# stvmsq/soc_project_stereo_matching

Hardware: AMD Instinct MI355X
Metric: Mdisp/s (W*H*D*paths/s; t_frame incl. H2D + D2H) (higher is better)
Workload: dtype u8

## Files before the change

### soc_project_stereo_matching_amd/csrc/sgm_aggregate_impl.hpp

```cpp
#pragma once
#include "sgm_common.hpp"

#ifndef SGM_AGG_PF
#define SGM_AGG_PF 2
#endif
#ifndef SGM_ANOM_PF
#define SGM_ANOM_PF 4
#endif
#ifndef SGM_AGG_HBURST
#define SGM_AGG_HBURST 1
#endif
#ifndef SGM_AGG_PF_HL
#define SGM_AGG_PF_HL 4
#endif


struct AggArgs {
    const uint8_t* img;
    const uint32_t* census_l;
    const uint32_t* census_r;
    const uint8_t* cost;
    int dmin;
    const uint16_t* lut;
    uint8_t* planes;
// ... 146 lines not shown
static __device__ __forceinline__ us2 pk_min_tree(const us2 (&v)[N])
{
    if constexpr (!FAST || N < 3) {
        us2 m = v[0];
#pragma unroll
        for (int j = 1; j < N; ++j) m = pk_min(m, v[j]);
        return m;
    } else {
        us2 m = pk_min3_f16(v[0], v[1], v[2]);
        int j = 3;
#pragma unroll
        for (; j + 1 < N; j += 2) m = pk_min3_f16(m, v[j], v[j + 1]);
        if (j < N) m = pk_min(m, v[j]);
        return m;
    }
}
template <int LPP>
static __device__ __forceinline__ unsigned row_allmin_pk(us2 m)
{
    unsigned r;
    asm("v_pk_min_u16 %0, %1, %1 op_sel:[0,1] op_sel_hi:[1,0]" : "=v"(r) : "v"(as_u(m)));
    return row_allmin<LPP>(r);
}
template <int DPL, bool PAD, int LPP, bool FAST = false>
static __device__ __forceinline__ unsigned agg_step_nn(unsigned cl, const CensusVec<DPL>& cv, int lim, bool border,
                                                       us2 (&Lp)[DPL / 2], unsigned mp, unsigned pen16, us2 p1v,
                                                       const us2 (&padmask)[DPL / 2], bool first_lane, bool last_lane,
                                                       unsigned (&sent)[2], CellVec<DPL>& packed_out)
{
    constexpr int NP = DPL / 2;
    const us2 p2v = as_p(pen16);
    const unsigned p1u = as_u(p1v);
    unsigned from_left, from_right;
    if (LPP >= 32) {
        from_left = sent[0] = dpp_mov<0x138 >(sent[0], as_u(Lp[NP - 1]));
        from_right = sent[1] = dpp_mov<0x130 >(sent[1], as_u(Lp[0]));
    } else {
        from_left = sent[0] = dpp_mov<DPP_ROW_SHR1>(sent[0], as_u(Lp[NP - 1]));
        from_right = sent[1] = dpp_mov<DPP_ROW_SHL1>(sent[1], as_u(Lp[0]));
    }
    if (LPP != 16) {
        from_left = first_lane ? 0x00FF00FFu : from_left;
        from_right = last_lane ? 0x00FF00FFu : from_right;
    }
    unsigned w[NP], md[NP];
#pragma unroll
    for (int j = 0; j < NP; ++j) {
        const unsigned below = (j == 0) ? from_left : as_u(Lp[j - 1]);
        const unsigned above = (j == NP - 1) ? from_right : as_u(Lp[j + 1]);
        const us2 dm1 = as_p(__builtin_amdgcn_alignbit(as_u(Lp[j]), below, 16) + p1u);
        const us2 dp1 = as_p(__builtin_amdgcn_alignbit(above, as_u(Lp[j]), 16) + p1u);
        us2 m;
        if constexpr (FAST) m = pk_min3_f16(dm1, dp1, Lp[j]);
        else m = pk_min(pk_min(dm1, dp1), Lp[j]);
        md[j] = as_u(pk_min(as_p(as_u(m) - mp), p2v));
        const unsigned lo = bcnt_acc(cl ^ cv.r[DPL - 1 - 2 * j], md[j]);
        w[j] = shl16_add((unsigned)__popc(cl ^ cv.r[DPL - 2 - 2 * j]), lo);
    }
    if (border) {
#pragma unroll
        for (int j = 0; j < NP; ++j) {
            const unsigned msk = (2 * j > lim ? 0xFFFFu : 0u) | (2 * j + 1 > lim ? 0xFFFF0000u : 0u);
            w[j] = (w[j] & ~msk) | ((md[j] + 0x007F007Fu) & msk);
            if constexpr (FAST) w[j] &= 0x00FF00FFu;
        }
    }
    us2 Ln[NP];
#pragma unroll
    for (int j = 0; j < NP; ++j) {
        unsigned r = w[j];
        if constexpr (!FAST) r &= 0x00FF00FFu;
        if (PAD) r |= as_u(padmask[j]);
        Ln[j] = as_p(r);
    }
    const us2 m = pk_min_tree<NP, FAST>(Ln);
#pragma unroll
    for (int j = 0; j < NP; ++j) Lp[j] = Ln[j];
    pack_cells<DPL>(Ln, packed_out);
    return row_allmin_pk<LPP>(m);
}

enum { AGG_H = 0, AGG_V = 1, AGG_D = 2 };

template <int DPL, bool PAD, int LPP, int KIND, int NN, bool WIDE = false, bool VOL = false, bool PWO = false>
static __device__ __forceinline__ void agg_regular(const AggArgs& a, const AggFrame& fr, const unsigned short* lut_s,
                                                   const unsigned* lut32_s, int dir, int grp)
{
    constexpr int NP = DPL / 2;
    constexpr int PF = (LPP >= 32) ? SGM_AGG_PF_HL : SGM_AGG_PF;
    const int lane = threadIdx.x;
    const int dx = a.dx[dir], dy = a.dy[dir];
    const int W = a.W, H = a.H, Dp = a.Dp;
    const bool fwd = (dx == 1 && dy == 0) || (dx == 0 && dy == 1) || (dx == 1 && dy == 1) || (dx == -1 && dy == 1);
    const int s = fwd ? 1 : -1;
    const int rows = a.row_end - a.row_begin;
    const int skip = (KIND == AGG_H) ? 0 : (fwd ? a.row_begin : H - a.row_end);
    const bool import_state = skip > 0;
    const int nlines = (KIND == AGG_H) ? rows : a.line_lo[dir] + a.line_n[dir];
    constexpr bool pwo = PWO;
    bool wrapped = false;
    const int nsteps = (KIND == AGG_H) ? W - 1 : (import_state ? rows : rows - 1);
    if (KIND == AGG_D && W < 2) return;

    constexpr int LPW = 64 / LPP;
    const int sub = lane & (LPP - 1);
    const bool first_lane = (sub == 0), last_lane = (sub == LPP - 1);
    int line = ((KIND == AGG_H) ? 0 : a.line_lo[dir]) + grp * LPW + lane / LPP;
    bool store_ok = line < nlines;
    if (!store_ok) line = nlines - 1;
    if (KIND == AGG_D && line == a.anom_line[dir]) {
        store_ok = false;
        line = (line == 0) ? 1 : line - 1;
    }
    const unsigned lane_off = (unsigned)(sub * DPL);
    uint8_t* const plane = fr.planes + (size_t)dir * a.plane_bytes;

    us2 padmask[NP];
#pragma unroll
    for (int j = 0; j < NP; ++j) {
        const unsigned lo = ((int)lane_off + 2 * j >= a.D) ? 0x00FFu : 0u;
        const unsigned hi = ((int)lane_off + 2 * j + 1 >= a.D) ? 0x00FF0000u : 0u;
        padmask[j] = as_p(lo | hi);
    }

    unsigned p, off;
    int x;
    unsigned rowpix = 0, rowoff = 0, pcol = 0, col = 0;
    int dstep_p = 0, dstep_off = 0;
    if (KIND == AGG_H) {
        x = fwd ? 0 : W - 1;
        p = (unsigned)((a.row_begin + line) * W + x);
        dstep_p = s; dstep_off = s * Dp;
    } else if (KIND == AGG_V) {
        x = line;
        const int r = fwd ? a.row_begin - (import_state ? 1 : 0) : a.row_end - 1 + (import_state ? 1 : 0);
        p = (unsigned)(r * W + line);
        dstep_p = s * W; dstep_off = s * W * Dp;
    } else {
        rowpix = (unsigned)(fwd ? 0 : (H - 1) * W);
        rowoff = rowpix * (unsigned)Dp;
        pcol = col = (unsigned)line;
        x = line;
        p = rowpix + pcol;
        dstep_p = s * W; dstep_off = s * W * Dp;
    }
    off = p * (unsigned)Dp + lane_off;
    const int col_step = (dx == dy) ? s : -s;
    const unsigned wrap_at = (col_step > 0) ? (unsigned)(W - 1) : 0u, wrap_to = (col_step > 0) ? 0u : (unsigned)(W - 1);
    const unsigned pstep_n = (unsigned)(dstep_p + col_step), pstep_w = (unsigned)(dstep_p - col_step * (W - 1));
    const unsigned ostep_n = pstep_n * (unsigned)Dp, ostep_w = pstep_w * (unsigned)Dp;
    const int back = a.dmin + (int)lane_off + DPL - 1;
    const int lim_bias = a.dmin + (int)lane_off;

    auto advance = [&]() {
        if (KIND == AGG_H) {
            p += (unsigned)dstep_p;
            off += (unsigned)dstep_off;
            x += s;
        } else if (KIND == AGG_V) {
            p += (unsigned)dstep_p;
            off += (unsigned)dstep_off;
        } else if (WIDE) {
            const bool wrap = (pcol == wrap_at);
            if constexpr (PWO) wrapped = wrapped || wrap;
            pcol = wrap ? wrap_to : pcol + (unsigned)col_step;
            p += wrap ? pstep_w : pstep_n;
            off += wrap ? ostep_w : ostep_n;
            x = (int)pcol;
        } else {
            const bool wr = (col == (unsigned)(W - 1));
            const bool wl = !wr && (col == 0);
            pcol = wr ? 0u : (wl ? (unsigned)(W - 1) : pcol + (unsigned)col_step);
            col = ((wr ? 0u : (wl ? (unsigned)(W - 1) : col)) + (unsigned)col_step) & 0xFFFFu;
            rowpix += (unsigned)dstep_p;
            rowoff += (unsigned)dstep_off;
            p = rowpix + pcol;
            x = (int)pcol;
            off = rowoff + __umul24(pcol, (unsigned)Dp) + lane_off;
        }
    };
    const unsigned cbias = (unsigned)(a.dmin + Dp - back);
    const char* const crb = reinterpret_cast<const char*>(fr.census_r - (a.dmin + Dp));
    const char* const clb_base = reinterpret_cast<const char*>(fr.census_l);
    auto fetch = [&](CensusVec<DPL>& cv, unsigned& cl, uint8_t& g) {
        if constexpr (VOL) {
            load_volume<DPL>(fr.cost + off, cv);
            cl = 0;
        } else {
            load_census<DPL>(reinterpret_cast<const uint32_t*>(crb + (size_t)((p + cbias) << 2)), cv);
            cl = *reinterpret_cast<const uint32_t*>(clb_base + (size_t)(p << 2));
        }
        g = fr.img[p];
    };

    if (KIND == AGG_D)
        for (int i = 0; i + 1 < skip; ++i) advance();

    us2 Lp[NP];
    unsigned min_prev;
    int g_prev;
    if (import_state) {
        CellVec<DPL> c0;
        load_cells<DPL>(plane + off, c0);
        g_prev = fr.img[p];
#pragma unroll
        for (int j = 0; j < NP; ++j) {
            const unsigned w = c0.w[j >> 1];
            Lp[j] = as_p(__builtin_amdgcn_perm(w, w, (j & 1) ? 0x0c030c02u : 0x0c010c00u));
        }
        us2 m = Lp[0];
#pragma unroll
        for (int j = 1; j < NP; ++j) m = pk_min(m, Lp[j]);
        min_prev = row_allmin<LPP>(min(as_u(m) & 0xFFFFu, as_u(m) >> 16));
    } else {
        CensusVec<DPL> cv;
        unsigned cl;
        uint8_t g0;
        fetch(cv, cl, g0);
        g_prev = g0;
        const int lim = x - lim_bias;
        if constexpr (VOL) volume_costs<DPL>(cv, Lp);
        else census_costs<DPL>(cl, cv, lim, true, Lp);
        if (PAD) {
#pragma unroll
            for (int j = 0; j < NP; ++j) Lp[j] = as_p(as_u(Lp[j]) | as_u(padmask[j]));
        }
        us2 m = Lp[0];
#pragma unroll
        for (int j = 1; j < NP; ++j) m = pk_min(m, Lp[j]);
        min_prev = row_allmin<LPP>(min(as_u(m) & 0xFFFFu, as_u(m) >> 16));
        if (store_ok && !pwo) {
            CellVec<DPL> o;
            pack_cells<DPL>(Lp, o);
            store_cells<DPL>(plane + off, o);
        }
    }

    CensusVec<DPL> cb[PF];
    unsigned clb[PF];
    uint8_t gb[PF];
    int limb[PF];
    unsigned ob[PF];
    bool wb[PF];
#pragma unroll
    for (int u = 0; u < PF; ++u) {
        gb[u] = 0; ob[u] = off; clb[u] = 0; limb[u] = 0; wb[u] = false;
#pragma unroll
        for (int i = 0; i < DPL; ++i) cb[u].r[i] = 0;
        if (1 + u <= nsteps) {
            advance();
            ob[u] = off;
            if constexpr (PWO) wb[u] = wrapped;
            limb[u] = x - lim_bias;
            fetch(cb[u], clb[u], gb[u]);
        }
    }
    const us2 p1v = splat((unsigned)a.p1);
    unsigned sent[2] = {0x00FF00FFu, 0x00FF00FFu};
    if constexpr (NN) min_prev |= min_prev << 16;

    auto step = [&](int u, bool refill, CellVec<DPL>* defer = nullptr, unsigned* defer_o = nullptr) {
        const int g = (int)gb[u];
        const int lim = limb[u];
        const unsigned o = ob[u];
        const bool st_ok = store_ok && (!pwo || wb[u]);
        const unsigned dg = __builtin_amdgcn_sad_u8((unsigned)g, (unsigned)g_prev, 0u);
        CellVec<DPL> packed;
        if constexpr (NN) {
            min_prev = agg_step_nn<DPL, PAD, LPP, NN == 2>(clb[u], cb[u], lim, __any(lim < DPL - 1) != 0, Lp, min_prev, lut32_s[dg], p1v,
                                                  padmask, first_lane, last_lane, sent, packed);
            if (refill) {
                advance();
                ob[u] = off;
                if constexpr (PWO) wb[u] = wrapped;
                limb[u] = x - lim_bias;
                fetch(cb[u], clb[u], gb[u]);
            }
        } else {
            us2 C[NP];
            if constexpr (VOL) volume_costs<DPL>(cb[u], C);
            else census_costs<DPL>(clb[u], cb[u], lim, __any(lim < DPL - 1) != 0, C);
            if (refill) {
                advance();
                ob[u] = off;
                if constexpr (PWO) wb[u] = wrapped;
                limb[u] = x - lim_bias;
                fetch(cb[u], clb[u], gb[u]);
            }
            min_prev = agg_step<DPL, PAD, LPP>(C, Lp, min_prev, lut_s[dg], p1v, padmask, first_lane, last_lane, packed);
        }
        g_prev = g;
        if (defer) { *defer = packed; *defer_o = o; }
        else if (st_ok) store_cells<DPL>(plane + o, packed);
    };
    __builtin_amdgcn_s_waitcnt(0x0F70);
    int k0 = 1;
    if constexpr (KIND == AGG_H && NN != 0 && SGM_AGG_HBURST > 1 && SGM_AGG_HBURST % PF == 0) {
        constexpr int HB = SGM_AGG_HBURST;
        for (; k0 + HB + PF - 1 <= nsteps; k0 += HB) {
            CellVec<DPL> pk[HB];
            unsigned po[HB];
#pragma unroll
            for (int j = 0; j < HB; ++j) step(j % PF, true, &pk[j], &po[j]);
            if (store_ok) {
#pragma unroll
                for (int j = 0; j < HB; ++j) store_cells<DPL>(plane + po[j], pk[j]);
            }
        }
    }
    for (; k0 + 2 * PF - 1 <= nsteps; k0 += PF) {
#pragma unroll
        for (int u = 0; u < PF; ++u) step(u, true);
    }
    for (; k0 <= nsteps; k0 += PF) {
#pragma unroll
        for (int u = 0; u < PF; ++u)
            if (k0 + u <= nsteps) step(u, k0 + u + PF <= nsteps);
    }
}

template <int DPL, bool PAD, int LPP, int NN, bool VOL = false>
static __device__ __forceinline__ void agg_anomalous(const AggArgs& a, const AggFrame& fr, const unsigned short* lut_s,
                                                     const unsigned* lut32_s, int dir)
{
    static_assert(!(NN && VOL), "the volume-fed lines run the generic step");
    constexpr int NP = DPL / 2;
    constexpr int NW = (DPL + 3) / 4;
    const int lane = threadIdx.x;
    const int dx = a.dx[dir], dy = a.dy[dir];
    const int W = a.W, H = a.H, Dp = a.Dp;
    const bool fwd = (dx == 1 && dy == 1) || (dx == -1 && dy == 1);
    const int s = fwd ? 1 : -1;
    const int diag_step = s * (W + ((dx == dy) ? 1 : -1));
    const int col_step = (dx == dy) ? s : -s;
    const int nsteps = H - 1;
    const long long npx = (long long)W * H;
    const int line = a.anom_line[dir];
    const int slot = dir - 4;
    const bool store_ok = lane < LPP;
    const int sub = lane & (LPP - 1);
    const bool first_lane = (sub == 0), last_lane = (sub == LPP - 1);
    const unsigned lane_off = (unsigned)(sub * DPL);
    uint8_t* const plane = fr.planes + (size_t)dir * a.plane_bytes;
    uint8_t* const extras = fr.extras + (size_t)slot * H * Dp + lane_off;

    us2 padmask[NP];
#pragma unroll
    for (int j = 0; j < NP; ++j) {
        const unsigned lo = ((int)lane_off + 2 * j >= a.D) ? 0x00FFu : 0u;
        const unsigned hi = ((int)lane_off + 2 * j + 1 >= a.D) ? 0x00FF0000u : 0u;
        padmask[j] = as_p(lo | hi);
    }
    auto ghost_zero = [&](int k) {
        if (store_ok && a.ghost_zero) {
            int gc = line + dx * k;
            if (gc >= W) gc -= W;
            if (gc < 0) gc += W;
            const int gr = fwd ? k : H - 1 - k;
            if (gr >= a.row_begin && gr < a.row_end) {
// ... 103 lines not shown
            if (refill) {
                advance();
                fetch(u);
            }
        } else {
            us2 C[NP];
            if constexpr (VOL) volume_costs<DPL>(cb[u], C);
            else census_costs<DPL>(clb[u], cb[u], limb[u], true, C);
            if (refill) {
                advance();
                fetch(u);
            }
            min_prev = agg_step<DPL, PAD, LPP>(C, Lp, min_prev, lut_s[dg], p1v, padmask, first_lane, last_lane, packed);
        }
        g_prev = g;
        if (store_ok) store_cells<DPL>(extras + (size_t)k * Dp, packed);
        ghost_zero(k);
    };
    __builtin_amdgcn_s_waitcnt(0x0F70);
    int k0 = 1;
    for (; k0 + 2 * PF - 1 <= n_live; k0 += PF) {
#pragma unroll
        for (int u = 0; u < PF; ++u) step(u, k0 + u, true);
    }
    for (; k0 <= n_live; k0 += PF) {
#pragma unroll
        for (int u = 0; u < PF; ++u)
            if (k0 + u <= n_live) step(u, k0 + u, k0 + u + PF <= n_live);
    }
    for (int k = n_live + 1; k <= nsteps; ++k) ghost_zero(k);
}

template <int DP> struct anom_layout   { static constexpr int lpp = (DP % 128 == 0) ? 64 : (DP == 64 ? 32 : 16), dpl = DP / lpp; };
template <int DP> struct anom_layout16 { static constexpr int lpp = 16, dpl = DP / 16; };

template <bool VOL>
static __device__ __forceinline__ AggFrame agg_frame(const AggArgs& a, int frame)
{
    AggFrame fr;
    fr.img = a.img + (size_t)frame * a.W * a.H;
    fr.census_l = a.census_l + (size_t)frame * a.W * a.H;
    fr.census_r = a.census_r + (size_t)frame * a.W * a.H;
    fr.cost = VOL ? a.cost + (size_t)frame * a.W * a.H * a.Dp : nullptr;
    fr.planes = a.planes + (size_t)frame * 8 * a.plane_bytes;
    fr.extras = a.extras + (size_t)frame * 4 * a.H * a.Dp;
    return fr;
}

template <int DPL, bool PAD, int LPP, int NN, bool VOL>
__global__ __launch_bounds__(64) void sgm_aggregate_anom_k(const AggArgs a)
{
    __shared__ unsigned short lut_s[256];
    __shared__ unsigned lut32_s[256];
    const int lane = threadIdx.x;
#pragma unroll
    for (int i = 0; i < 4; ++i) {
        const unsigned pen = a.lut[lane * 4 + i];
        lut_s[lane * 4 + i] = (unsigned short)pen;
        lut32_s[lane * 4 + i] = pen * 0x00010001u;
    }
    __syncthreads();
    const AggFrame fr = agg_frame<VOL>(a, blockIdx.x % a.B);
    agg_anomalous<DPL, PAD, LPP, NN, VOL>(a, fr, lut_s, lut32_s, 4 + blockIdx.x / a.B);
}
#ifdef SGM_CLOCK_PROBE
static __device__ unsigned long long g_sgm_agg_clock[2];
#endif

template <int DPL, bool PAD, int LPP, int HL, int NN, bool VOL = false>
__global__ __launch_bounds__(64) void sgm_aggregate_k(const AggArgs a)
{
#ifdef SGM_CLOCK_PROBE
    const unsigned long long clk0 = __builtin_amdgcn_s_memtime(), rt0 = __builtin_amdgcn_s_memrealtime();
    struct ClockProbe {
        unsigned long long c0, r0;
        __device__ ~ClockProbe() {
            if (blockIdx.x == 0 && threadIdx.x == 0) {
                g_sgm_agg_clock[0] = __builtin_amdgcn_s_memtime() - c0;
                g_sgm_agg_clock[1] = __builtin_amdgcn_s_memrealtime() - r0;
            }
        }
    } probe{clk0, rt0};
#endif
    __shared__ unsigned short lut_s[256];
    __shared__ unsigned lut32_s[256];
    const int lane = threadIdx.x;
#pragma unroll
    for (int i = 0; i < 4; ++i) {
        const unsigned pen = a.lut[lane * 4 + i];
        lut_s[lane * 4 + i] = (unsigned short)pen;
        lut32_s[lane * 4 + i] = pen * 0x00010001u;
    }
    __syncthreads();

    int frame, b;
    const int n_anom = a.anom_inline ? 4 : 0;
    if (a.strips > 1) {
        const int xcd = blockIdx.x & 7;
        frame = xcd % a.B;
        const int sub = xcd / a.B;
        int q = blockIdx.x >> 3;
        b = -1;
        for (int dd = 0; dd <= 8; ++dd) {
            const int d = dd == 0 ? 8 : dd - 1;
            const int begin = a.block_begin[d];
            const int n = (d < 8 ? a.block_begin[d + 1] : begin + n_anom) - begin;
            const int lo = sub * n / a.strips, share = (sub + 1) * n / a.strips - lo;
            if (q < share) { b = begin + lo + q; break; }
            q -= share;
        }
        if (b < 0) return;
    } else {
        frame = blockIdx.x % a.B;
        b = blockIdx.x / a.B;
        b = b < n_anom ? a.block_begin[8] + b : b - n_anom;
    }
    const AggFrame fr = agg_frame<VOL>(a, frame);
    if constexpr (NN != 0 && !VOL) {
        if (b >= a.block_begin[8]) {
            using AL = anom_layout<DPL * LPP>;
            agg_anomalous<AL::dpl, PAD, AL::lpp, 1, false>(a, fr, lut_s, lut32_s, 4 + (b - a.block_begin[8]));
            return;
        }
    }
    int dir = 0;
    while (dir + 1 < a.ndirs && b >= a.block_begin[dir + 1]) ++dir;
    const int grp = b - a.block_begin[dir];
    if (a.dy[dir] == 0) __builtin_amdgcn_s_setprio(3);
    if (a.dy[dir] == 0) {
        if constexpr (HL != 0) agg_regular<DPL * LPP / HL, PAD, HL, AGG_H, NN, false, VOL>(a, fr, lut_s, lut32_s, dir, grp);
        else               agg_regular<DPL, PAD, LPP, AGG_H, NN, false, VOL>(a, fr, lut_s, lut32_s, dir, grp);
    }
    else if (a.dx[dir] == 0) agg_regular<DPL, PAD, LPP, AGG_V, NN, false, VOL>(a, fr, lut_s, lut32_s, dir, grp);
    else if (a.W > a.H) {
        if constexpr (NN != 0 && !VOL) {
            if ((a.post_wrap_mask >> dir) & 1) {
                agg_regular<DPL, PAD, LPP, AGG_D, NN, true, VOL, true>(a, fr, lut_s, lut32_s, dir, grp);
                return;
            }
        }
        agg_regular<DPL, PAD, LPP, AGG_D, NN, true, VOL>(a, fr, lut_s, lut32_s, dir, grp);
    }
    else                     agg_regular<DPL, PAD, LPP, AGG_D, NN, false, VOL>(a, fr, lut_s, lut32_s, dir, grp);
}

template <int DPL, int LPP, int HL, int NN>
static bool launch_aggregate_hl(const AggArgs& a, int blocks, bool pad, hipStream_t st)
{
    constexpr int per = (HL != 0) ? DPL * LPP / HL : DPL;
    constexpr bool ok = (HL == 0) || ((DPL * LPP) % HL == 0 && (per == 2 || per == 4 || per == 8 || per == 16) && HL != LPP);
    if constexpr (ok) {
        if (pad) hipLaunchKernelGGL((sgm_aggregate_k<DPL, true, LPP, HL, NN>), dim3(blocks), dim3(64), 0, st, a);
        else     hipLaunchKernelGGL((sgm_aggregate_k<DPL, false, LPP, HL, NN>), dim3(blocks), dim3(64), 0, st, a);
        return true;
    }
    return false;
}
template <int DPL, int LPP, int NN>
static void launch_aggregate(const AggArgs& a, int blocks, bool pad, int hl, hipStream_t st)
{
    if constexpr (NN) {
        if (hl == 64 && launch_aggregate_hl<DPL, LPP, 64, NN>(a, blocks, pad, st)) return;
        if (hl == 32 && launch_aggregate_hl<DPL, LPP, 32, NN>(a, blocks, pad, st)) return;
        if (hl == 16 && launch_aggregate_hl<DPL, LPP, 16, NN>(a, blocks, pad, st)) return;
    }
    launch_aggregate_hl<DPL, LPP, 0, NN>(a, blocks, pad, st);
}

template <int NN>
static bool launch_aggregate_key(int lpp, int dpl, const AggArgs& a, int blocks, bool pad, int hl, hipStream_t st)
{
    switch (lpp * 100 + dpl) {
    case 1602: launch_aggregate<2, 16, NN>(a, blocks, pad, hl, st); return true;
    case 1604: launch_aggregate<4, 16, NN>(a, blocks, pad, hl, st); return true;
    case 1608: launch_aggregate<8, 16, NN>(a, blocks, pad, hl, st); return true;
    case 1612: launch_aggregate<12, 16, NN>(a, blocks, pad, hl, st); return true;
    case 1616: launch_aggregate<16, 16, NN>(a, blocks, pad, hl, st); return true;
    case 1632: launch_aggregate<32, 16, NN>(a, blocks, pad, hl, st); return true;
    default: break;
    }
    if constexpr (NN) {
        switch (lpp * 100 + dpl) {
        case 804: launch_aggregate<4, 8, NN>(a, blocks, pad, hl, st); return true;
        case 808: launch_aggregate<8, 8, NN>(a, blocks, pad, hl, st); return true;
        case 816: launch_aggregate<16, 8, NN>(a, blocks, pad, hl, st); return true;
        default: break;
        }
    }
    return false;
}
```

### soc_project_stereo_matching_amd/csrc/sgm_host.c

```c
#include "../../include/sgm_mi355x.h"
#include "sgm_device.h"

#include <math.h>
#include <stddef.h>
#include <stdio.h>
#include <stdlib.h>
#include <string.h>

#define SGM_VERSION_STRING "sgm_mi355x 0.3 (gfx950, hand-written HIP)"
#define CENSUS_FRONT_SLACK ((size_t)(65535 + SGM_MAX_DISPARITY_RANGE + 8 + 63) / 64 * 64 * 4)

#define TIMING_RING 64
enum { T_CENSUS, T_COST, T_AGGREGATE, T_SUM, T_WTA, T_LRCHECK, T_SPECKLE, T_MEDIAN, T_COUNT };
#define M_END T_COUNT
#define M_SUM_BEGIN (T_COUNT + 1)
#define MARKS_PER_MATCH (T_COUNT + 2)
static const char* const k_stage_names[T_COUNT] = {"census", "cost", "aggregate", "sum", "wta", "lrcheck", "speckle", "median"};

static const int k_dir_dx[8] = {1, -1, 0, 0, 1, -1, 1, -1};
static const int k_dir_dy[8] = {0, 0, 1, -1, 1, -1, -1, 1};

typedef struct { void* p; size_t cap; } sgm_buf;
typedef struct { void* dst; const void* src; size_t bytes; } handover;

typedef enum { S_ZERO, S_STORED, S_IN_PLANES, S_IN_PLANES_ADDS } sum_where;
typedef struct { sum_where where; bool up_missing; } sum_state;

typedef struct {
    float lambda, sigma;
    int iters, keep_invalid;
    float tab[SGM_REFINE_MAX_ITERS][256];
} refine_params;

struct sgm_instance {
    int device;
    void* stream;
    void* sum_stream;
    void* post_stream;
    void *ev_agg, *ev_sum, *ev_post;
    int overlap_post;
    bool sum_pending;
    bool post_pending;
    void* tail_stream;
    int cu_first[3], cu_count[3];
    int up_rows;
    sgm_buf d_up_scratch;
    sgm_buf d_left_keep;
    unsigned up_gen;
    int up_key[5];
    int last_up_rows;
    int env_upsum, env_upsum_rows, env_upsum_wgs;
    int env_lanes, env_hl, env_agg_fast, env_fused;
    bool stage_prio[3];
    int* h_status;
    void* timer;
    int timing;
    int keep_stages;
    int honor_num_paths;
    int census_w, census_h;
    int census_kind;
    int reference_view;
    int pixel_bits_req;
    int pixel_bits;
    int fill_req;
    bool fill_on;
    int refine_req;
    bool refine_on;
    int reference_statics;
    int batch;
    int read_frame;
    int tile_begin, tile_end;
    const void* tile_left;

    bool initialized;
    sum_state S;
    int fused_wta;
    SGMOption opt;
    sgmd_geom g;
    sgmd_paths paths;
    int need_plane_memset;
    int row_cap;
    float last_ms[T_COUNT];
    bool have_ms;
    int ring_next, ring_pending;
    double sum_ms[T_COUNT], min_ms[T_COUNT];
    long n_timed;

    int plane_row_lo, plane_rows;
    int tab_W, tab_H, tab_ndirs, tab_p1, tab_p2;
    sgm_buf d_left, d_right, d_census_l, d_census_r_alloc, d_cost, d_planes_alloc, d_extras, d_S;
    void *d_census_r, *d_planes;
    sgm_buf d_disp, d_disp_r, d_labels, d_sizes, d_lut, d_row_extras, d_row_count;
    sgm_buf d_snap_wta, d_snap_lr, d_snap_speckle, d_totals, d_median_scratch;
// ... 615 lines not shown
    const int bw = 64, bh = 16;
    for (int r = s->g.row_begin / bh; r <= (s->g.row_end - 1) / bh; ++r) memset(need + (size_t)r * bx, 1, (size_t)bx);
    if (s->paths.ndirs > 4) {
        const int back = s->g.dmin + s->g.Dp + 64;
        for (int d = 4; d < 8; ++d) {
            const int cnt = walk_line(W, H, k_dir_dx[d], k_dir_dy[d], s->paths.anom_line[d], pix);
            for (int k = 0; k < cnt; ++k) {
                const int y = pix[k] / W, x = pix[k] % W;
                const int c0 = (x - back < 0 ? 0 : x - back) / bw, c1 = x / bw;
                memset(need + (size_t)(y / bh) * bx + c0, 1, (size_t)(c1 - c0 + 1));
                if (x - back < 0 && y > 0) need[(size_t)((y - 1) / bh) * bx + bx - 1] = 1;
            }
        }
    }
    free(pix);
    const bool ok = reserve(s, &s->d_census_need, n, 0) && sgmd_h2d_async(s->device, s->stream, s->d_census_need.p, need, n) == 0 && sync_streams(s) == 0;
    free(need);
    if (!ok) FAIL("uploading the census block map failed");
    memcpy(s->need_key, key, sizeof key);
    return true;
}

#define ROW_EXTRAS_MAX ((size_t)1 << 24)

static bool upload_tables(sgm_instance* s)
{
    const int W = s->g.W, H = s->g.H;
    uint16_t lut[256];
    build_p2_table(s->opt.p1, s->opt.p2_init, lut);

    int32_t* pix = (int32_t*)malloc(sizeof(int32_t) * (size_t)(W > H ? W : H));
    int* count = (int*)calloc((size_t)H, sizeof(int));
    int32_t* visits = (int32_t*)malloc(sizeof(int32_t) * 4 * (size_t)H);
    if (!pix || !count || !visits) { free(pix); free(count); free(visits); FAIL("out of host memory"); }
    for (int i = 0; i < 4 * H; ++i) visits[i] = -1;
    if (s->paths.ndirs > 4) {
        for (int slot = 0; slot < 4; ++slot) {
            const int d = 4 + slot;
            const int n = walk_line(W, H, k_dir_dx[d], k_dir_dy[d], s->paths.anom_line[d], pix);
            for (int k = 0; k < n; ++k) {
                visits[slot * H + k] = pix[k];
                count[pix[k] / W]++;
            }
        }
    }
    int cap = 1;
    for (int r = 0; r < H; ++r) if (count[r] > cap) cap = count[r];
    if ((size_t)H * cap > ROW_EXTRAS_MAX) {
        free(pix); free(count); free(visits);
        FAIL("a frame %d wide and %d rows tall is not supported: its anomalous lines visit one row %d times (a frame one pixel wide "
             "is accepted up to 4096 rows)", W, H, cap);
    }
    sgmd_row_extra* table = (sgmd_row_extra*)calloc((size_t)H * cap, sizeof *table);
    if (!table) { free(pix); free(count); free(visits); FAIL("out of host memory"); }
    memset(count, 0, sizeof(int) * (size_t)H);
    for (int slot = 0; slot < 4; ++slot)
        for (int k = 0; k < H; ++k) {
            const int32_t p = visits[slot * H + k];
            if (p < 0) continue;
            const int r = p / W, c = p % W;
            table[(size_t)r * cap + count[r]].col_slot = c | (slot << 16);
            table[(size_t)r * cap + count[r]].step = k;
            count[r]++;
        }

    const buf_request tables[] = {{&s->d_row_extras, sizeof *table * (size_t)H * cap, 0}, {&s->d_row_count, sizeof(int) * (size_t)H, 0}};
    s->row_cap = cap;
    const bool ok = reserve_all(s, tables, 2, BUF_LAZY_DRAIN) && sgmd_h2d_async(s->device, s->stream, s->d_row_extras.p, table, sizeof *table * (size_t)H * cap) == 0 &&
         sgmd_h2d_async(s->device, s->stream, s->d_row_count.p, count, sizeof(int) * (size_t)H) == 0 &&
         sgmd_h2d_async(s->device, s->stream, s->d_lut.p, lut, sizeof lut) == 0 &&
         sync_streams(s) == 0;
    free(table); free(visits); free(count); free(pix);
    if (!ok) FAIL("uploading path tables failed");
    return true;
}

static bool ensure_buffers(sgm_instance* s)
{
    const int dev = s->device;
    const size_t px = batch_px(s);
    if (!buf_holds(&s->d_disp, px * 4)) {
        const size_t img = image_bytes(s);
        const buf_request images[] = {{&s->d_left, img, 0}, {&s->d_right, img, 0}, {&s->d_census_l, px * 4, 0},
                                      {&s->d_census_r_alloc, CENSUS_FRONT_SLACK + px * 4, 0}};
        const buf_request maps[] = {{&s->d_disp, px * 4, 0}, {&s->d_disp_r, px * 4, 0}, {&s->d_labels, px * 4, 0}, {&s->d_sizes, px * 4, 0},
                                    {&s->d_totals, px * 4, 0}, {&s->d_lut, 512, 0}, {&s->d_snap_wta, px * 4, 0}, {&s->d_snap_lr, px * 4, 0},
                                    {&s->d_snap_speckle, px * 4, 0}, {&s->h_left, img, BUF_PINNED}, {&s->h_right, img, BUF_PINNED},
                                    {&s->h_disp, px * 4, BUF_PINNED}};
        sync_streams(s);
        const sgm_buf old_l = s->d_census_l, old_r = s->d_census_r_alloc;
        s->d_census_l = s->d_census_r_alloc = (sgm_buf){NULL, 0};
        free_device_buffers(s);
        int rc = reserve_all(s, images, 4, BUF_LAZY_DRAIN) ? 0 : -1;
        if (rc == 0) s->d_census_r = (char*)s->d_census_r_alloc.p + CENSUS_FRONT_SLACK;
        if (rc == 0) rc |= sgmd_memset_async(dev, s->stream, s->d_census_l.p, 0, px * 4);
        if (rc == 0) rc |= sgmd_memset_async(dev, s->stream, s->d_census_r_alloc.p, 0, CENSUS_FRONT_SLACK + px * 4);
        if (rc == 0 && s->reference_statics && old_l.p && old_r.p) {
            rc |= sgmd_d2d_async(dev, s->stream, s->d_census_l.p, old_l.p, old_l.cap);
            rc |= sgmd_d2d_async(dev, s->stream, s->d_census_r, (char*)old_r.p + CENSUS_FRONT_SLACK, old_l.cap);
        }
        if (rc == 0) rc |= sgmd_stream_sync(dev, s->stream);
        sgmd_free(dev, old_l.p);
        sgmd_free(dev, old_r.p);
        if (rc != 0 || !reserve_all(s, maps, 12, BUF_LAZY_DRAIN)) {
            free_device_buffers(s);
            FAIL("device allocation failed for %dx%dx%d", s->g.W, s->g.H, s->g.D);
        }
    }
    if (wide_pixels(s)) {
        const size_t img = image_bytes(s);
        const buf_request wide[] = {{&s->d_left, img, 0}, {&s->d_right, img, 0}, {&s->h_left, img, BUF_PINNED}, {&s->h_right, img, BUF_PINNED},
                                    {&s->d_g8_l, px, 0}, {&s->d_g8_r, px, 0}};
        if (!reserve_all(s, wide, 6, 0)) FAIL("device allocation failed for the %d-bit images of %dx%d", s->pixel_bits, s->g.W, s->g.H);
    }
    const bool tiled = row_tiled(s);
    s->plane_row_lo = tiled && s->g.row_begin > 0 ? s->g.row_begin - 1 : 0;
    const int row_hi = tiled && s->g.row_end < s->g.H ? s->g.row_end + 1 : s->g.H;
    s->plane_rows = row_hi - s->plane_row_lo;
    s->plane_bytes = (size_t)s->plane_rows * s->g.W * s->g.Dp;
    const size_t need = (size_t)s->g.B * 8 * s->plane_bytes;
    if (!reserve(s, &s->d_planes_alloc, need, 0))
        FAIL("device allocation failed for the path-cost planes of %dx%dx%d (%zu bytes)", s->g.W, s->g.H, s->g.D, need);
    s->d_planes = (void*)((uintptr_t)s->d_planes_alloc.p - (uintptr_t)s->plane_row_lo * s->g.W * s->g.Dp);
    return true;
}

static int ensure_S(sgm_instance* s)
{
    const size_t need = batch_px(s) * s->g.Dp * 2;
    if (buf_holds(&s->d_S, need)) return 0;
    if (reserve(s, &s->d_S, need, BUF_ZERO) &&
        (!s->sum_stream || sgmd_stream_sync(s->device, s->stream) == 0))
        return 0;
    fprintf(stderr, "sgm_mi355x: device allocation failed for the aggregated-cost volume (%zu bytes)\n", need);
    return -1;
}

static int ensure_cost(sgm_instance* s)
{
    const size_t need = batch_px(s) * s->g.Dp;
    if (reserve(s, &s->d_cost, need, 0)) return 0;
    fprintf(stderr, "sgm_mi355x: device allocation failed for the cost volume (%zu bytes)\n", need);
    return -1;
}

static int ensure_fill(sgm_instance* s)
{
    const size_t px = batch_px(s);
    const buf_request maps[] = {{&s->d_fill_class, px, 0}, {&s->d_fill_map, px * sizeof(float), 0}};
    if (reserve_all(s, maps, 2, 0)) return 0;
    fprintf(stderr, "sgm_mi355x: device allocation failed for the hole-filling maps (%zu pixels)\n", px);
    return -1;
}

static int ensure_refine(sgm_instance* s)
{
    const size_t px = batch_px(s);
    const buf_request maps[] = {{&s->d_rf_u, px * 4, 0}, {&s->d_rf_v, px * 4, 0}, {&s->d_rf_q, px * 4, 0}, {&s->d_rf_conf, px * 2, 0},
                                {&s->d_rf_guide[0], px, 0}, {&s->d_rf_guide[1], px, 0}};
    if (reserve_all(s, maps, 6, 0)) return 0;
    fprintf(stderr, "sgm_mi355x: device allocation failed for the refinement maps (%zu pixels)\n", px);
    return -1;
}

static int refine_passes(sgm_instance* s, void* st, void* disp, const void* conf, const void* guide, const refine_params* p)
{
    int rc = 0;
// ... 1427 lines not shown
```

Baseline: 1.883 million.

## Share right-census window across lanes via LDS in vertical/diagonal aggregation

For vertical and wide-diagonal aggregation paths, each wave now cooperatively loads one contiguous run of right-image census words per step (one 16-byte vector per lane) into shared memory. Each lane then reads its DPL-wide disparity window from LDS instead of issuing its own overlapping global gathers. Diagonals that wrap across the image edge use a second run. The aim is to cut redundant global/L2 traffic for overlapping census windows. In exchange it adds LDS writes, reads and wave barriers per step, shrinks lut_s when NN is set, and needs extra back slack on the census buffer for over-reads.

Result: faster. 1.950 million (median of 6 runs) (+3.5%).

```diff
diff --git a/soc_project_stereo_matching_amd/csrc/sgm_aggregate_impl.hpp b/soc_project_stereo_matching_amd/csrc/sgm_aggregate_impl.hpp
--- a/soc_project_stereo_matching_amd/csrc/sgm_aggregate_impl.hpp
+++ b/soc_project_stereo_matching_amd/csrc/sgm_aggregate_impl.hpp
@@ -252,11 +252,21 @@
 
 enum { AGG_H = 0, AGG_V = 1, AGG_D = 2 };
 
+template <int DPL, int LPP> struct agg_feed {
+    static constexpr int LPW = 64 / LPP;
+    static constexpr int RUNW = (DPL * LPP + LPW + 2 + 3) & ~3;
+    static constexpr bool on = DPL >= 16 && LPP <= 16 && RUNW / 4 <= 64;
+    static constexpr int BASE_DOWN = 16;
+};
+
 template <int DPL, bool PAD, int LPP, int KIND, int NN, bool WIDE = false, bool VOL = false, bool PWO = false>
 static __device__ __forceinline__ void agg_regular(const AggArgs& a, const AggFrame& fr, const unsigned short* lut_s,
-                                                   const unsigned* lut32_s, int dir, int grp)
+                                                   const unsigned* lut32_s, unsigned* feed_s, int dir, int grp)
 {
     constexpr int NP = DPL / 2;
+    using FD = agg_feed<DPL, LPP>;
+    constexpr bool FEED = FD::on && NN != 0 && !VOL && !PWO && (KIND == AGG_V || (KIND == AGG_D && WIDE));
+    constexpr int NRUN = (KIND == AGG_D) ? 2 : 1;
     constexpr int PF = (LPP >= 32) ? SGM_AGG_PF_HL : SGM_AGG_PF;
     const int lane = threadIdx.x;
     const int dx = a.dx[dir], dy = a.dy[dir];
@@ -275,13 +285,15 @@
     constexpr int LPW = 64 / LPP;
     const int sub = lane & (LPP - 1);
     const bool first_lane = (sub == 0), last_lane = (sub == LPP - 1);
-    int line = ((KIND == AGG_H) ? 0 : a.line_lo[dir]) + grp * LPW + lane / LPP;
+    const int line0 = ((KIND == AGG_H) ? 0 : a.line_lo[dir]) + grp * LPW;
+    int line = line0 + lane / LPP;
     bool store_ok = line < nlines;
     if (!store_ok) line = nlines - 1;
     if (KIND == AGG_D && line == a.anom_line[dir]) {
         store_ok = false;
         line = (line == 0) ? 1 : line - 1;
     }
+    const int feed_col = line - line0 + 1;
     const unsigned lane_off = (unsigned)(sub * DPL);
     uint8_t* const plane = fr.planes + (size_t)dir * a.plane_bytes;
 
@@ -297,6 +309,7 @@
     int x;
     unsigned rowpix = 0, rowoff = 0, pcol = 0, col = 0;
     int dstep_p = 0, dstep_off = 0;
+    unsigned frow = 0, fcol = 0;
     if (KIND == AGG_H) {
         x = fwd ? 0 : W - 1;
         p = (unsigned)((a.row_begin + line) * W + x);
@@ -306,6 +319,8 @@
         const int r = fwd ? a.row_begin - (import_state ? 1 : 0) : a.row_end - 1 + (import_state ? 1 : 0);
         p = (unsigned)(r * W + line);
         dstep_p = s * W; dstep_off = s * W * Dp;
+        frow = (unsigned)(r * W);
+        fcol = (unsigned)(line0 - 1);
     } else {
         rowpix = (unsigned)(fwd ? 0 : (H - 1) * W);
         rowoff = rowpix * (unsigned)Dp;
@@ -313,6 +328,8 @@
         x = line;
         p = rowpix + pcol;
         dstep_p = s * W; dstep_off = s * W * Dp;
+        frow = rowpix;
+        fcol = (unsigned)(line0 > 0 ? line0 - 1 : W - 1);
     }
     off = p * (unsigned)Dp + lane_off;
     const int col_step = (dx == dy) ? s : -s;
@@ -330,7 +347,12 @@
         } else if (KIND == AGG_V) {
             p += (unsigned)dstep_p;
             off += (unsigned)dstep_off;
+            if constexpr (FEED) frow += (unsigned)dstep_p;
         } else if (WIDE) {
+            if constexpr (FEED) {
+                fcol = (fcol == wrap_at) ? wrap_to : fcol + (unsigned)col_step;
+                frow += (unsigned)dstep_p;
+            }
             const bool wrap = (pcol == wrap_at);
             if constexpr (PWO) wrapped = wrapped || wrap;
             pcol = wrap ? wrap_to : pcol + (unsigned)col_step;
@@ -362,6 +384,23 @@
         }
         g = fr.img[p];
     };
+    struct FeedRegs { unsigned w[NRUN][4]; };
+    const char* const frb = reinterpret_cast<const char*>(fr.census_r - (a.dmin + Dp + FD::BASE_DOWN));
+    auto fetch_feed = [&](FeedRegs& f, unsigned& cl, uint8_t& g) {
+        struct __attribute__((packed, aligned(4))) u4 { unsigned a, b, c, d; };
+        const unsigned wa = frow + fcol + (unsigned)(FD::BASE_DOWN + 1);
+#pragma unroll
+        for (int r = 0; r < NRUN; ++r) {
+            const unsigned wr = (r == 1 && (int)fcol + FD::LPW + 1 >= W) ? wa - (unsigned)W : wa;
+            const unsigned grp4 = min((unsigned)lane, (unsigned)(FD::RUNW / 4 - 1));
+            const u4 t = *reinterpret_cast<const u4*>(frb + (size_t)((wr + 4 * grp4) << 2));
+            f.w[r][0] = t.a; f.w[r][1] = t.b; f.w[r][2] = t.c; f.w[r][3] = t.d;
+        }
+        cl = *reinterpret_cast<const uint32_t*>(clb_base + (size_t)(p << 2));
+        g = fr.img[p];
+    };
+    const unsigned feed_rd = (unsigned)(feed_col + Dp - (int)lane_off - DPL);
+    const int feed_wrap_lim = feed_col - lim_bias;
 
     if (KIND == AGG_D)
         for (int i = 0; i + 1 < skip; ++i) advance();
@@ -407,6 +446,7 @@
     }
 
     CensusVec<DPL> cb[PF];
+    FeedRegs fb[PF];
     unsigned clb[PF];
     uint8_t gb[PF];
     int limb[PF];
@@ -417,14 +457,33 @@
         gb[u] = 0; ob[u] = off; clb[u] = 0; limb[u] = 0; wb[u] = false;
 #pragma unroll
         for (int i = 0; i < DPL; ++i) cb[u].r[i] = 0;
+        if constexpr (FEED) {
+#pragma unroll
+            for (int i = 0; i < NRUN * 4; ++i) (&fb[u].w[0][0])[i] = 0;
+        }
         if (1 + u <= nsteps) {
             advance();
             ob[u] = off;
             if constexpr (PWO) wb[u] = wrapped;
             limb[u] = x - lim_bias;
-            fetch(cb[u], clb[u], gb[u]);
-        }
-    }
+            if constexpr (FEED) fetch_feed(fb[u], clb[u], gb[u]);
+            else fetch(cb[u], clb[u], gb[u]);
+        }
+    }
+    auto feed_window = [&](const FeedRegs& f, int lim, CensusVec<DPL>& cv) {
+#pragma unroll
+        for (int r = 0; r < NRUN; ++r)
+            if (lane < FD::RUNW / 4) {
+                uint4 t;
+                t.x = f.w[r][0]; t.y = f.w[r][1]; t.z = f.w[r][2]; t.w = f.w[r][3];
+                *reinterpret_cast<uint4*>(feed_s + r * FD::RUNW + 4 * lane) = t;
+            }
+        __builtin_amdgcn_wave_barrier();
+        const unsigned* const src = feed_s + feed_rd + ((NRUN == 2 && lim < feed_wrap_lim) ? (unsigned)FD::RUNW : 0u);
+#pragma unroll
+        for (int i = 0; i < DPL; ++i) cv.r[i] = src[i];
+        __builtin_amdgcn_wave_barrier();
+    };
     const us2 p1v = splat((unsigned)a.p1);
     unsigned sent[2] = {0x00FF00FFu, 0x00FF00FFu};
     if constexpr (NN) min_prev |= min_prev << 16;
@@ -437,6 +496,7 @@
         const unsigned dg = __builtin_amdgcn_sad_u8((unsigned)g, (unsigned)g_prev, 0u);
         CellVec<DPL> packed;
         if constexpr (NN) {
+            if constexpr (FEED) feed_window(fb[u], lim, cb[u]);
             min_prev = agg_step_nn<DPL, PAD, LPP, NN == 2>(clb[u], cb[u], lim, __any(lim < DPL - 1) != 0, Lp, min_prev, lut32_s[dg], p1v,
                                                   padmask, first_lane, last_lane, sent, packed);
             if (refill) {
@@ -444,7 +504,8 @@
                 ob[u] = off;
                 if constexpr (PWO) wb[u] = wrapped;
                 limb[u] = x - lim_bias;
-                fetch(cb[u], clb[u], gb[u]);
+                if constexpr (FEED) fetch_feed(fb[u], clb[u], gb[u]);
+                else fetch(cb[u], clb[u], gb[u]);
             }
         } else {
             us2 C[NP];
@@ -714,13 +775,15 @@
         }
     } probe{clk0, rt0};
 #endif
-    __shared__ unsigned short lut_s[256];
+    constexpr bool FEEDS = NN != 0 && !VOL && agg_feed<DPL, LPP>::on;
+    __shared__ unsigned short lut_s[NN != 0 ? 2 : 256];
     __shared__ unsigned lut32_s[256];
+    __shared__ __attribute__((aligned(16))) unsigned feed_s[FEEDS ? 2 * agg_feed<DPL, LPP>::RUNW : 4];
     const int lane = threadIdx.x;
 #pragma unroll
     for (int i = 0; i < 4; ++i) {
         const unsigned pen = a.lut[lane * 4 + i];
-        lut_s[lane * 4 + i] = (unsigned short)pen;
+        if constexpr (NN == 0) lut_s[lane * 4 + i] = (unsigned short)pen;
         lut32_s[lane * 4 + i] = pen * 0x00010001u;
     }
     __syncthreads();
@@ -760,20 +823,20 @@
     const int grp = b - a.block_begin[dir];
     if (a.dy[dir] == 0) __builtin_amdgcn_s_setprio(3);
     if (a.dy[dir] == 0) {
-        if constexpr (HL != 0) agg_regular<DPL * LPP / HL, PAD, HL, AGG_H, NN, false, VOL>(a, fr, lut_s, lut32_s, dir, grp);
-        else               agg_regular<DPL, PAD, LPP, AGG_H, NN, false, VOL>(a, fr, lut_s, lut32_s, dir, grp);
-    }
-    else if (a.dx[dir] == 0) agg_regular<DPL, PAD, LPP, AGG_V, NN, false, VOL>(a, fr, lut_s, lut32_s, dir, grp);
+        if constexpr (HL != 0) agg_regular<DPL * LPP / HL, PAD, HL, AGG_H, NN, false, VOL>(a, fr, lut_s, lut32_s, feed_s, dir, grp);
+        else               agg_regular<DPL, PAD, LPP, AGG_H, NN, false, VOL>(a, fr, lut_s, lut32_s, feed_s, dir, grp);
+    }
+    else if (a.dx[dir] == 0) agg_regular<DPL, PAD, LPP, AGG_V, NN, false, VOL>(a, fr, lut_s, lut32_s, feed_s, dir, grp);
     else if (a.W > a.H) {
         if constexpr (NN != 0 && !VOL) {
             if ((a.post_wrap_mask >> dir) & 1) {
-                agg_regular<DPL, PAD, LPP, AGG_D, NN, true, VOL, true>(a, fr, lut_s, lut32_s, dir, grp);
+                agg_regular<DPL, PAD, LPP, AGG_D, NN, true, VOL, true>(a, fr, lut_s, lut32_s, feed_s, dir, grp);
                 return;
             }
         }
-        agg_regular<DPL, PAD, LPP, AGG_D, NN, true, VOL>(a, fr, lut_s, lut32_s, dir, grp);
-    }
-    else                     agg_regular<DPL, PAD, LPP, AGG_D, NN, false, VOL>(a, fr, lut_s, lut32_s, dir, grp);
+        agg_regular<DPL, PAD, LPP, AGG_D, NN, true, VOL>(a, fr, lut_s, lut32_s, feed_s, dir, grp);
+    }
+    else                     agg_regular<DPL, PAD, LPP, AGG_D, NN, false, VOL>(a, fr, lut_s, lut32_s, feed_s, dir, grp);
 }
 
 template <int DPL, int LPP, int HL, int NN>
diff --git a/soc_project_stereo_matching_amd/csrc/sgm_host.c b/soc_project_stereo_matching_amd/csrc/sgm_host.c
--- a/soc_project_stereo_matching_amd/csrc/sgm_host.c
+++ b/soc_project_stereo_matching_amd/csrc/sgm_host.c
@@ -9,6 +9,7 @@
 
 #define SGM_VERSION_STRING "sgm_mi355x 0.3 (gfx950, hand-written HIP)"
 #define CENSUS_FRONT_SLACK ((size_t)(65535 + SGM_MAX_DISPARITY_RANGE + 8 + 63) / 64 * 64 * 4)
+#define CENSUS_BACK_SLACK ((size_t)64)
 
 #define TIMING_RING 64
 enum { T_CENSUS, T_COST, T_AGGREGATE, T_SUM, T_WTA, T_LRCHECK, T_SPECKLE, T_MEDIAN, T_COUNT };
@@ -790,7 +791,7 @@
     if (!buf_holds(&s->d_disp, px * 4)) {
         const size_t img = image_bytes(s);
         const buf_request images[] = {{&s->d_left, img, 0}, {&s->d_right, img, 0}, {&s->d_census_l, px * 4, 0},
-                                      {&s->d_census_r_alloc, CENSUS_FRONT_SLACK + px * 4, 0}};
+                                      {&s->d_census_r_alloc, CENSUS_FRONT_SLACK + px * 4 + CENSUS_BACK_SLACK, 0}};
         const buf_request maps[] = {{&s->d_disp, px * 4, 0}, {&s->d_disp_r, px * 4, 0}, {&s->d_labels, px * 4, 0}, {&s->d_sizes, px * 4, 0},
                                     {&s->d_totals, px * 4, 0}, {&s->d_lut, 512, 0}, {&s->d_snap_wta, px * 4, 0}, {&s->d_snap_lr, px * 4, 0},
                                     {&s->d_snap_speckle, px * 4, 0}, {&s->h_left, img, BUF_PINNED}, {&s->h_right, img, BUF_PINNED},
```
